# df07/mcp-raytracer

Hardware: AMD Instinct MI355X
Metric: Msamples/sec (w×h×spp/s) Cornell 800×800 spp=256 @1/2/4/8 GPU (higher is better)
Workload: dtype f64

## Files before the change

mcp-raytracer_amd/csrc/pt_kernel.hpp:

```cpp
#pragma once

#include <hip/hip_runtime.h>

#include <cstdint>
#include <type_traits>

#include "rt_math.hpp"
#include "scene.hpp"

namespace rt {

struct DevScene {
    const RtTNode* __restrict__ tnodes;
    const RtPrim* __restrict__ prims;
    const RtPrim* __restrict__ gprims;
    const RtPre* __restrict__ gpre;
    int32_t n_pre;
    const RtExact* __restrict__ xrec;
    int32_t off_xrec;
    const int32_t* __restrict__ tprims;
    const float4* __restrict__ tsph;
    const RtMat* __restrict__ mats;
    const RtLight* __restrict__ lights;
    const RtLight* __restrict__ glights;
// ... 2036 lines not shown
}
__device__ __forceinline__ void item_pixel(const RtRegion& reg, int tiles_x, double rtx, int mt, int l, int& i,
                                           int& j) {
    const int gt = reg.tile_group + mt * reg.tile_groups;
    const int ty = udiv(gt, tiles_x, rtx);
    i = reg.x + (gt - ty * tiles_x) * kTile + (l & (kTile - 1));
    j = reg.y + ty * kTile + (l / kTile);
}
template <class SB>
__device__ __forceinline__ bool slot_pixel(const SB& sb, const RtRegion& reg, int tiles_x, double rtx, int endX,
                                           int endY, int a, int& i, int& j) {
    int ls = a;
    if (sb.act) {
        if (a >= sb.slots) return false;
        ls = sb.act[a];
        __builtin_amdgcn_s_waitcnt(0x0F70);
    }
    item_pixel(reg, tiles_x, rtx, sb.tile0 + (ls >> 6), ls & 63, i, j);
    return i < endX && j < endY;
}

struct PhaseRow {
    int32_t s0, chunk, nch, base;
    double rnch;
    int32_t pad[2];
};
__device__ __forceinline__ void phase_table_init(const SampleBuf& sb, PhaseRow* tab) {
    const int t = threadIdx.x;
    if (t < kMaxPhases) {
        PhaseRow r;
        r.s0 = sb.s0[t];
        r.chunk = sb.chunk[t];
        r.nch = sb.nch[t];
        r.base = t < sb.n_phases ? sb.item_base[t] : 0x7fffffff;
        r.rnch = sb.rnch[t];
        r.pad[0] = r.pad[1] = 0;
        tab[t] = r;
    }
    __syncthreads();
}
__device__ __forceinline__ void item_decode(const SampleBuf& sb, const PhaseRow* tab, int u, int& tl, int& l, int& s,
                                            int& s_end) {
    int ph = 0;
    for (int q = 1; q < sb.n_phases; ++q) ph += u >= tab[q].base ? 1 : 0;
    const PhaseRow r = tab[ph];
    const int v = u - r.base;
    const int q = v >> 6;
    l = v & 63;
    tl = udiv(q, r.nch, r.rnch);
    const int ch = q - tl * r.nch;
    s = r.s0 + ch * r.chunk;
    s_end = s + r.chunk;
}

__device__ __forceinline__ void first_pool(const SampleBuf& sb, int& pool_next, int& pool_end, bool& exhausted) {
    const int gw = (int)(blockIdx.x * (blockDim.x / kWave) + threadIdx.x / kWave);
    pool_next = gw * sb.pool;
    pool_end = min(pool_next + sb.pool, sb.n_items);
    exhausted = pool_next >= sb.n_items;
}
__device__ __forceinline__ void take_pool(const RenderOut& out, const SampleBuf& sb, int lane, int& pool_next,
                                          int& pool_end, bool& exhausted) {
    int base = 0;
    if (lane == 0) base = (int)atomicAdd(out.tile_counter, (unsigned)sb.pool);
    base = __builtin_amdgcn_readfirstlane(__shfl(base, 0, 64)) + (int)(gridDim.x * (blockDim.x / kWave)) * sb.pool;
    if (base >= sb.n_items) {
        exhausted = true;
        return;
    }
    pool_next = base;
    pool_end = min(base + sb.pool, sb.n_items);
}

struct KernArgs {
    DevScene S0;
    RtRegion reg;
    RenderOut out;
    int tiles_x;
    SampleBuf sb;
};
__device__ __forceinline__ const KernArgs& kern_args() {
    KArgPtr p = (KArgPtr)__builtin_amdgcn_kernarg_segment_ptr();
    asm volatile("" : "+s"(p));
    return *(const KernArgs*)p;
}

template <class Real, bool EMIT, int INSTR, int TRAV, int LDSS>
__global__ __launch_bounds__(kBlockChunk) void pt_chunk_kernel(DevScene S0, RtRegion reg, RenderOut out,
                                                                        int tiles_x, SampleBuf sb) {
    constexpr bool COUNT = INSTR == 1;
    constexpr bool PROF = INSTR == 2;
    extern __shared__ int lds_stack[];
    const RtCamera& C0 = S0.cam;
    __shared__ PhaseRow ptab[kMaxPhases];
    phase_table_init(sb, ptab);
    const DevScene S = scene_prologue<LDSS>(S0, lds_stack);
    const int lane = threadIdx.x & (kWave - 1);
    StackT<LDSS>* stk = reinterpret_cast<StackT<LDSS>*>(lds_stack) + threadIdx.x;
    const int endX = min(reg.x + reg.width, C0.width);
    const int endY = min(reg.y + reg.height, C0.height);
    const int n_items = sb.n_items;

    uint32_t cnt[CT_WORDS];
    if (COUNT) {
#pragma unroll
        for (int k = 0; k < CT_WORDS; ++k) cnt[k] = 0;
    }
    unsigned long long st_err = 0;
    __shared__ unsigned long long prof_lds[PROF ? kProfWaves * kProfSlot : 1];
    Prof pf;
    prof_init<PROF>(pf, prof_lds, lane);

    int pool_next, pool_end;
    bool exhausted;
    first_pool(sb, pool_next, pool_end, exhausted);
    int slot = -1;
    int s = 0, s_end = 0, i = 0, j = 0;
    uint32_t pix = 0;
    V3 pc = v3(0, 0, 0);
    bool new_path = false;
    Path<EMIT> P;
    const double rtx = 1.0 / (double)tiles_x;
    constexpr bool RS = trav_fast(TRAV) && INSTR != 1;
    FastWalk<Real> W;
    bool walking = false;
    LaneBounces lb;

#define PK_SB (kern_args().sb)
#define PK_REG (kern_args().reg)
#define PK_OUT (kern_args().out)
#define PK_S (scene_view<LDSS>(kern_args().S0, lds_stack))
    while (true) {
        const unsigned long long need = __ballot(slot < 0);
        const int n_need = __popcll(need);
        if (n_need != 0 && !exhausted && (n_need >= PK_SB.refill_min || __ballot(slot >= 0) == 0ull)) {
            if (pool_next >= pool_end) take_pool(PK_OUT, PK_SB, lane, pool_next, pool_end, exhausted);
            if (!exhausted) {
                const int take = min(n_need, pool_end - pool_next);
                const int rank = __builtin_amdgcn_mbcnt_hi((uint32_t)(need >> 32),
                                                           __builtin_amdgcn_mbcnt_lo((uint32_t)need, 0u));
                if (slot < 0 && rank < take) {
                    int tl, l, s1, e1;
                    item_decode(PK_SB, ptab, pool_next + rank, tl, l, s1, e1);
                    if (slot_pixel(PK_SB, PK_REG, tiles_x, rtx, endX, endY, tl * 64 + l, i, j)) {
                        slot = tl * 64 + l;
                        s = s1;
                        s_end = e1;
                        pix = (uint32_t)j * (uint32_t)C0.width + (uint32_t)i;
                        pc = pixel_center<Real>(cam_opaque(), i, j);
                        new_path = true;
                    }
                }
                pool_next += take;
            }
        }
        psec<PROF>(pf, PR_TILE);
        if (__ballot(slot >= 0) == 0ull) {
            if (exhausted) break;
            continue;
        }
        if constexpr (RS) {
            auto finish_sample = [&](V3 c) {
                rec_put<false>(PK_SB, (size_t)s * PK_SB.stride_s + (size_t)slot * PK_SB.stride_slot, c,
                               P.bounces | rec_err_bits(PK_SB.err_in_rec, st_err), lb, PK_OUT.stats);
                ++s;
                if (s < s_end) new_path = true;
                else slot = -1;
            };
            const RtCamera& C = cam_opaque();
            prof_trip<PROF>(pf);
            if (slot >= 0 && !walking) {
                if (new_path) {
                    path_begin<Real, EMIT>(C, P, pc, pix, (uint32_t)(PK_SB.s_base + s));
                    new_path = false;
                    psec<PROF>(pf, PR_NEWPATH);
                }
                V3 c;
                if (path_pre<Real, EMIT, PROF>(C, P, pf, c)) {
                    finish_sample(c);
                } else {
                    fast_walk_begin<Real, COUNT>(PK_S, P.o, P.d, W, cnt);
                    walking = true;
                }
            }
            psec<PROF>(pf, PR_RR);
            const bool was_walking = walking;
            fast_walk_rounds<Real, COUNT, TRAV == TRAV_FAST_DEFER, PROF, kStackStride, LDSS == 0>(
                PK_S, P.o, P.d, W, walking, stk, PK_SB.min_ready, exhausted, cnt, &pf);
            psec<PROF>(pf, PR_HIT);
            if (was_walking && !walking) {
                fast_walk_resolve<Real, COUNT>(PK_S, P.o, P.d, W, cnt);
                V3 c;
                if (path_post<Real, EMIT, COUNT, PROF>(PK_S, C, P, W.best, W.best_t, cnt, st_err, pf, c))
                    finish_sample(c);
            }
            psec<PROF>(pf, PR_ACC);
        } else if (slot >= 0) {
            const RtCamera& C = cam_opaque();
            prof_trip<PROF>(pf);
            if (new_path) {
                path_begin<Real, EMIT>(C, P, pc, pix, (uint32_t)(PK_SB.s_base + s));
                new_path = false;
                psec<PROF>(pf, PR_NEWPATH);
            }
            V3 c;
            if (path_trip<Real, EMIT, COUNT, PROF, TRAV>(PK_S, C, P, stk, cnt, st_err, pf, c)) {
                rec_put<false>(PK_SB, (size_t)s * PK_SB.stride_s + (size_t)slot * PK_SB.stride_slot, c,
                               P.bounces | rec_err_bits(PK_SB.err_in_rec, st_err), lb, PK_OUT.stats);
                if (COUNT) {
                    cnt[CT_SAMPLES]++;
                    cnt[CT_BOUNCES] += (uint32_t)P.bounces;
                }
                ++s;
                if (s < s_end) new_path = true;
                else slot = -1;
                psec<PROF>(pf, PR_ACC);
            }
        }
    }
    PixStats st;
    lb.to(st);
    publish_stats(out, st, st_err, lane);
    publish_counters<COUNT, PROF>(out, cnt, pf, lane);
#undef PK_SB
#undef PK_REG
#undef PK_OUT
#undef PK_S
}

#ifndef RT_POOL_K
#define RT_POOL_K 152
#endif
#ifndef RT_POOL_PROF
#define RT_POOL_PROF 0
#endif
constexpr int kPoolK = RT_POOL_K;
constexpr int kBlockPool = 1024;
constexpr int kPoolGroups = 3;
static_assert(kPoolK >= kWave && kPoolK <= 256, "pool slots: one full wave, u8 queue entries");
constexpr size_t kPoolWaveBytes = ((size_t)kPoolK * (kPoolGroups * 16 + 8) + 2 * kPoolK + 15) / 16 * 16;
constexpr int kPoolClog2Bits = 3;
constexpr int kPoolMaxChunk = 1 << ((1 << kPoolClog2Bits) - 1);
__device__ __forceinline__ float pool_meta(int phase, int clog2, int mat) {
    return __uint_as_float((uint32_t)((phase + 2) & 0xff) | ((uint32_t)clog2 << 8) | ((uint32_t)mat << 11));
}
__device__ __forceinline__ int meta_phase(float m) { return (int)(__float_as_uint(m) & 0xffu) - 2; }
__device__ __forceinline__ int meta_clog2(float m) { return (int)((__float_as_uint(m) >> 8) & 7u); }
__device__ __forceinline__ int meta_mat(float m) { return (int)(__float_as_uint(m) >> 11); }
__device__ __forceinline__ float pool_hs(int hf16, int s) { return __uint_as_float(((uint32_t)hf16 & 0xffffu) | ((uint32_t)s << 16)); }
__device__ __forceinline__ int hs_s(float v) { return (int)(__float_as_uint(v) >> 16); }
__device__ __forceinline__ int hs_hf(float v) { return (int)(__float_as_uint(v) & 0xffffu); }
__device__ __forceinline__ int item_end(int s, int clog2) { return ((s >> clog2) + 1) << clog2; }
constexpr size_t pool_lds_bytes() { return (size_t)(kBlockPool / kWave) * kPoolWaveBytes; }
enum : int { PH_NEW = -1, PH_ITEM = -2 };

__device__ __forceinline__ void stack_push(uint8_t* q, bool top, int& cnt, bool want, int k) {
    const unsigned long long m = __ballot(want);
    if (want) {
        const int r = __builtin_amdgcn_mbcnt_hi((uint32_t)(m >> 32), __builtin_amdgcn_mbcnt_lo((uint32_t)m, 0u));
        q[top ? kPoolK - 1 - (cnt + r) : cnt + r] = (uint8_t)k;
    }
    cnt += __popcll(m);
}

struct KernArgsPrimary {
    KernArgs args;
    const uint2* ptab;
};
__device__ __forceinline__ const uint2* primary_table_opaque() {
    KArgPtr p = (KArgPtr)__builtin_amdgcn_kernarg_segment_ptr();
    asm volatile("" : "+s"(p));
    return *(const uint2* const*)(p + offsetof(KernArgsPrimary, ptab));
}

template <class Real, int TRAV, int LDSS, bool PRIM>
__device__ __forceinline__ void pool_trips(DevScene S0, RtRegion reg, RenderOut out, int tiles_x, SampleBuf sb) {
    extern __shared__ int lds_stack[];
    const RtCamera& C0 = S0.cam;
    __shared__ PhaseRow ptab[kMaxPhases];
    phase_table_init(sb, ptab);
    const DevScene S = scene_prologue<LDSS>(S0, lds_stack);
    const int lane = threadIdx.x & (kWave - 1);
    StackT<LDSS>* stk = reinterpret_cast<StackT<LDSS>*>(lds_stack) + threadIdx.x;
    char* wpool = reinterpret_cast<char*>(lds_stack) + S0.lds_pool_off + (size_t)(threadIdx.x / kWave) * kPoolWaveBytes;
    float4* G = reinterpret_cast<float4*>(wpool);
    float2* G3 = reinterpret_cast<float2*>(wpool + (size_t)kPoolK * kPoolGroups * 16);
    uint8_t* qa = reinterpret_cast<uint8_t*>(wpool + (size_t)kPoolK * (kPoolGroups * 16 + 8));
    uint8_t* qd = qa + kPoolK;
    const int endX = min(reg.x + reg.width, C0.width);
    const int endY = min(reg.y + reg.height, C0.height);
    const int n_items = sb.n_items;
    const double rtx = 1.0 / (double)tiles_x;
    uint32_t* cnt = nullptr;
    unsigned long long st_err = 0;
    constexpr bool PP = RT_POOL_PROF;
    __shared__ unsigned long long prof_lds[PP ? kProfWaves * kProfSlot : 1];
    Prof pf;
    prof_init<PP>(pf, prof_lds, lane);

    for (int k = lane; k < kPoolK; k += kWave) {
        qa[k] = (uint8_t)k;
        G[k] = make_float4(0.f, 0.f, pool_meta(PH_ITEM, 0, 0), 0.f);
    }
    int a_cnt = kPoolK, d_cnt = 0;
    int dl_cnt = 0;
    int an_cnt = kPoolK, ac_cnt = 0;
    int pool_next, pool_end;
    bool exhausted;
    first_pool(sb, pool_next, pool_end, exhausted);

    LaneBounces lb;
    auto record = [&](V3 c, int bounces, int slot, int& s, int s_end, unsigned long long err = 0ull) -> int {
        if (!sb.err_in_rec) st_err |= err;
        rec_put<true>(sb, (size_t)s * sb.stride_s + (size_t)slot * sb.stride_slot, c,
                           bounces | (sb.err_in_rec ? (int)((uint32_t)err << kRecErrShift) : 0), lb, out.stats);
        ++s;
        return s < s_end ? PH_NEW : PH_ITEM;
    };

    while (a_cnt + d_cnt + dl_cnt > 0) {
        __asm__ volatile("" ::: "memory");
        prof_trip<PP>(pf);
        psec<PP>(pf, PR_ACC);
        const bool dtop = dl_cnt > d_cnt;
        const int dn = dtop ? dl_cnt : d_cnt;
        const bool atop = ac_cnt > an_cnt;
        const int an = atop ? ac_cnt : an_cnt;
        if (dn >= kWave || dn > an) {
            const int n = min(kWave, dn);
            int k = -1, phase = 0;
            if (lane < n) k = (int)qd[dtop ? kPoolK - dl_cnt + lane : d_cnt - n + lane];
            if (dtop) dl_cnt -= n;
            else d_cnt -= n;
            if (k >= 0) {
                const float4 g0 = G[k], g1 = G[kPoolK + k], g2 = G[2 * kPoolK + k];
                const float2 g3 = G3[k];
                Path<false> P;
                P.rng = (uint64_t)__float_as_uint(g0.x) | ((uint64_t)__float_as_uint(g0.y) << 32);
                P.bounces = meta_phase(g0.z);
                P.em_n = 0;
                P.o = V3{g1.x, g1.y, g1.z};
                P.d = V3{g2.x, g2.y, g2.z};
                P.T = V3{g2.w, g3.x, g3.y};
                const int hf = hs_hf(g0.w);
                const int h = hf & 0x3fff;
                const bool planar = (hf >> 14) & 1, front = (hf >> 15) & 1;
                const V3 att = ld3(S.mats[meta_mat(g0.z)].color);
                const int clog2 = meta_clog2(g0.z), slot = __float_as_int(g1.w);
                int s = hs_s(g0.w);
                const int s_end = item_end(s, clog2);
                phase = P.bounces;
                const RtCamera& C = cam_opaque();
                const bool dterm =
                    dtop ? shade_diffuse<Real, false, false, PP, 2>(S, C, P, h, planar, front, P.o, P.d, att, cnt, pf)
                         : shade_diffuse<Real, false, false, PP, 1>(S, C, P, h, planar, front, P.o, P.d, att, cnt, pf);
                if (dterm) {
                    const V3 c = mulv(ld3(S.mats[S.prims[h].mat].emitted), P.T);
                    phase = record(c, P.bounces, slot, s, s_end);
                }
                G[k] = make_float4(__uint_as_float((uint32_t)P.rng), __uint_as_float((uint32_t)(P.rng >> 32)),
                                   pool_meta(phase, clog2, 0), pool_hs(0, s));
                G[2 * kPoolK + k] = make_float4(P.d.x, P.d.y, P.d.z, P.T.x);
                G3[k] = make_float2(P.T.y, P.T.z);
            }
            stack_push(qa, false, an_cnt, k >= 0 && phase < 0, k);
            stack_push(qa, true, ac_cnt, k >= 0 && phase >= 0, k);
            a_cnt = an_cnt + ac_cnt;
        } else {
            const int n = min(kWave, an);
            int k = -1;
            if (lane < n) k = (int)qa[atop ? kPoolK - ac_cnt + lane : an_cnt - n + lane];
            if (atop) ac_cnt -= n;
            else an_cnt -= n;
            a_cnt -= n;
            float4 g0 = make_float4(0.f, 0.f, pool_meta(PH_ITEM, 0, 0), 0.f), g1 = g0, g2 = g0;
            float2 g3 = make_float2(0.f, 0.f);
            if (k >= 0) {
                g0 = G[k];
                g1 = G[kPoolK + k];
                g2 = G[2 * kPoolK + k];
                g3 = G3[k];
            }
            int phase = meta_phase(g0.z), clog2 = meta_clog2(g0.z), slot = __float_as_int(g1.w);
            int s = hs_s(g0.w);
            const unsigned long long need = __ballot(k >= 0 && phase == PH_ITEM);
            if (need != 0ull && !exhausted) {
                if (pool_next >= pool_end) take_pool(out, sb, lane, pool_next, pool_end, exhausted);
                if (!exhausted) {
                    const int take = min(__popcll(need), pool_end - pool_next);
                    const int rank = __builtin_amdgcn_mbcnt_hi((uint32_t)(need >> 32),
                                                               __builtin_amdgcn_mbcnt_lo((uint32_t)need, 0u));
                    if (k >= 0 && phase == PH_ITEM && rank < take) {
                        int tl, l, s1, e1, i, j;
                        item_decode(sb, ptab, pool_next + rank, tl, l, s1, e1);
                        if (slot_pixel(sb, reg, tiles_x, rtx, endX, endY, tl * 64 + l, i, j)) {
                            slot = tl * 64 + l;
                            s = s1;
                            clog2 = __builtin_ctz((uint32_t)(e1 - s1));
                            phase = PH_NEW;
                        }
                    }
                    pool_next += take;
                }
            }
            const bool keep = k >= 0 && (phase != PH_ITEM || !exhausted);
            bool to_d = false, d_light = false;
            if (k >= 0 && phase != PH_ITEM) {
                const RtCamera& C = cam_opaque();
                Path<false> P;
                uint2 prec = make_uint2(0u, 0u);
                if (phase == PH_NEW) {
                    int i, j;
                    slot_pixel(sb, reg, tiles_x, rtx, endX, endY, slot, i, j);
                    const uint32_t pix = (uint32_t)j * (uint32_t)C.width + (uint32_t)i;
                    if (PRIM) prec = primary_table_opaque()[pix];
                    path_begin<Real, false>(C, P, pixel_center<Real>(C, i, j), pix, (uint32_t)(sb.s_base + s));
                    if (PRIM) __builtin_amdgcn_s_waitcnt(0x0F70);
                } else {
                    P.rng = (uint64_t)__float_as_uint(g0.x) | ((uint64_t)__float_as_uint(g0.y) << 32);
                    P.o = V3{g1.x, g1.y, g1.z};
                    P.d = V3{g2.x, g2.y, g2.z};
                    P.T = V3{g2.w, g3.x, g3.y};
                    P.bounces = phase;
                    P.em_n = 0;
                }
                V3 c;
                psec<PP>(pf, PR_NEWPATH);
                bool term = path_pre<Real, false, PP>(C, P, pf, c);
                V3 att;
                int hf = 0, dmat = 0;
                unsigned long long err = 0ull;
                if (!term) {
                    const RayK<Real> ray = make_ray<Real>(P.o, P.d);
                    Real t;
                    int h;
                    if (PRIM && !atop) {
                        psec<PP>(pf, PR_TILE);
                        h = closest_hit_primary<Real, false>(S, ray, t, prec, cnt);
                    } else if (PP && TRAV == TRAV_BRUTE && C.n_prims <= kBruteMaxPrims)
                        h = closest_hit_brute_nf<Real, false>(S, C.n_prims, ray, t, lot_column(stk), cnt,
                                                              [&]() { psec<PP>(pf, PR_TILE); });
                    else
                        h = closest_hit_any<Real, false, TRAV>(S, C.n_prims, ray, t, stk, cnt);
                    psec<PP>(pf, PR_HIT);
                    if (h < 0) {
                        term = true;
                        c = miss_color<Real, false, PP>(C, P, err, pf);
                    } else {
                        V3 p, nrm, emitted, sdir;
                        bool front, planar;
                        const int kind = shade_hit<Real, false, false, PP>(S, P, h, t, cnt, pf, p, nrm, front,
                                                                              planar, emitted, att, sdir, &dmat);
                        if (kind == SC_NONE) {
                            term = true;
                            c = emitted;
                        } else {
                            ++P.bounces;
                            P.o = p;
                            if (kind == SC_SPEC) {
                                P.T = mulv(P.T, att);
                                P.d = sdir;
                            } else {
                                to_d = true;
                                P.d = nrm;
                                hf = h | (planar ? (1 << 14) : 0) | (front ? (1 << 15) : 0);
                                {
                                    uint64_t r = P.rng;
                                    const Real u0 = uniform<Real>(r);
                                    const Real rnd = S.mix_total == 1.0 ? u0 : u0 * (Real)S.mix_total;
                                    d_light = !(rnd < (Real)0.5 || C.n_lights == 0);
                                }
                            }
                        }
                    }
                }
                phase = term ? record(c, P.bounces, slot, s, item_end(s, clog2), err) : P.bounces;
                g0 = make_float4(__uint_as_float((uint32_t)P.rng), __uint_as_float((uint32_t)(P.rng >> 32)),
                                 pool_meta(phase, clog2, to_d ? dmat : 0), pool_hs(to_d ? hf : 0, s));
                g1 = make_float4(P.o.x, P.o.y, P.o.z, __int_as_float(slot));
                g2 = make_float4(P.d.x, P.d.y, P.d.z, P.T.x);
                g3 = make_float2(P.T.y, P.T.z);
            } else if (keep) {
                g0 = make_float4(0.f, 0.f, pool_meta(PH_ITEM, 0, 0), 0.f);
            }
            if (keep) {
                G[k] = g0;
                G[kPoolK + k] = g1;
                G[2 * kPoolK + k] = g2;
                G3[k] = g3;
            }
            stack_push(qa, false, an_cnt, keep && !to_d && phase < 0, k);
            stack_push(qa, true, ac_cnt, keep && !to_d && phase >= 0, k);
            a_cnt = an_cnt + ac_cnt;
            stack_push(qd, false, d_cnt, to_d && !d_light, k);
            stack_push(qd, true, dl_cnt, to_d && d_light, k);
        }
    }
    PixStats st;
    lb.to(st);
    publish_stats(out, st, st_err, lane);
    publish_counters<false, PP>(out, cnt, pf, lane);
}

template <class Real, int TRAV, int LDSS>
__global__ __launch_bounds__(kBlockPool) void pt_pool_kernel(DevScene S0, RtRegion reg, RenderOut out, int tiles_x,
                                                               SampleBuf sb) {
    pool_trips<Real, TRAV, LDSS, false>(S0, reg, out, tiles_x, sb);
}
template <class Real, int TRAV, int LDSS>
__global__ __launch_bounds__(kBlockPool) void pt_pool_primary_kernel(DevScene S0, RtRegion reg, RenderOut out,
                                                                       int tiles_x, SampleBuf sb, const uint2* ptab) {
    (void)ptab;
    pool_trips<Real, TRAV, LDSS, true>(S0, reg, out, tiles_x, sb);
}

}
```

Measured before the change: 13410.

## Merge diffuse and continuation path queues into one per-trip wave schedule

The wavefront pool loop used to run either a diffuse-shading batch or an active-path batch on each trip. Now a diffuse batch is topped up with continuing active paths so all lanes stay busy, and after diffuse shading those lanes go straight on to trace their next ray in the same trip. New-path fetching keeps its own batch type. The aim is fewer idle lanes and fewer loop trips, at the cost of more divergence within a wave and higher register pressure from the unified body.

Measured after the change: 13770 (median of 6 runs). 1.03x the previous value.

```diff
diff --git a/mcp-raytracer_amd/csrc/pt_kernel.hpp b/mcp-raytracer_amd/csrc/pt_kernel.hpp
--- a/mcp-raytracer_amd/csrc/pt_kernel.hpp
+++ b/mcp-raytracer_amd/csrc/pt_kernel.hpp
@@ -2362,8 +2362,7 @@
         qa[k] = (uint8_t)k;
         G[k] = make_float4(0.f, 0.f, pool_meta(PH_ITEM, 0, 0), 0.f);
     }
-    int a_cnt = kPoolK, d_cnt = 0;
-    int dl_cnt = 0;
+    int d_cnt = 0, dl_cnt = 0;
     int an_cnt = kPoolK, ac_cnt = 0;
     int pool_next, pool_end;
     bool exhausted;
@@ -2378,71 +2377,56 @@
         return s < s_end ? PH_NEW : PH_ITEM;
     };
 
-    while (a_cnt + d_cnt + dl_cnt > 0) {
+    enum : int { FR_N, FR_D, FR_NONE };
+    while (an_cnt + ac_cnt + d_cnt + dl_cnt > 0) {
         __asm__ volatile("" ::: "memory");
         prof_trip<PP>(pf);
         psec<PP>(pf, PR_ACC);
         const bool dtop = dl_cnt > d_cnt;
         const int dn = dtop ? dl_cnt : d_cnt;
-        const bool atop = ac_cnt > an_cnt;
-        const int an = atop ? ac_cnt : an_cnt;
-        if (dn >= kWave || dn > an) {
-            const int n = min(kWave, dn);
-            int k = -1, phase = 0;
-            if (lane < n) k = (int)qd[dtop ? kPoolK - dl_cnt + lane : d_cnt - n + lane];
-            if (dtop) dl_cnt -= n;
-            else d_cnt -= n;
-            if (k >= 0) {
-                const float4 g0 = G[k], g1 = G[kPoolK + k], g2 = G[2 * kPoolK + k];
-                const float2 g3 = G3[k];
-                Path<false> P;
-                P.rng = (uint64_t)__float_as_uint(g0.x) | ((uint64_t)__float_as_uint(g0.y) << 32);
-                P.bounces = meta_phase(g0.z);
-                P.em_n = 0;
-                P.o = V3{g1.x, g1.y, g1.z};
-                P.d = V3{g2.x, g2.y, g2.z};
-                P.T = V3{g2.w, g3.x, g3.y};
-                const int hf = hs_hf(g0.w);
-                const int h = hf & 0x3fff;
-                const bool planar = (hf >> 14) & 1, front = (hf >> 15) & 1;
-                const V3 att = ld3(S.mats[meta_mat(g0.z)].color);
-                const int clog2 = meta_clog2(g0.z), slot = __float_as_int(g1.w);
-                int s = hs_s(g0.w);
-                const int s_end = item_end(s, clog2);
-                phase = P.bounces;
-                const RtCamera& C = cam_opaque();
-                const bool dterm =
-                    dtop ? shade_diffuse<Real, false, false, PP, 2>(S, C, P, h, planar, front, P.o, P.d, att, cnt, pf)
-                         : shade_diffuse<Real, false, false, PP, 1>(S, C, P, h, planar, front, P.o, P.d, att, cnt, pf);
-                if (dterm) {
-                    const V3 c = mulv(ld3(S.mats[S.prims[h].mat].emitted), P.T);
-                    phase = record(c, P.bounces, slot, s, s_end);
-                }
-                G[k] = make_float4(__uint_as_float((uint32_t)P.rng), __uint_as_float((uint32_t)(P.rng >> 32)),
-                                   pool_meta(phase, clog2, 0), pool_hs(0, s));
-                G[2 * kPoolK + k] = make_float4(P.d.x, P.d.y, P.d.z, P.T.x);
-                G3[k] = make_float2(P.T.y, P.T.z);
-            }
-            stack_push(qa, false, an_cnt, k >= 0 && phase < 0, k);
-            stack_push(qa, true, ac_cnt, k >= 0 && phase >= 0, k);
-            a_cnt = an_cnt + ac_cnt;
+        const int fr = dn >= kWave       ? FR_D
+                       : ac_cnt >= kWave ? FR_NONE
+                       : an_cnt >= kWave ? FR_N
+                       : dn > 0          ? FR_D
+                       : an_cnt > 0      ? FR_N
+                                         : FR_NONE;
+        int k = -1;
+        int nd = 0;
+        if (fr == FR_D) {
+            nd = min(kWave, dn);
+            const int na = min(kWave - nd, ac_cnt);
+            if (lane < nd) k = (int)qd[dtop ? kPoolK - dl_cnt + lane : d_cnt - nd + lane];
+            else if (lane < nd + na) k = (int)qa[kPoolK - ac_cnt + lane - nd];
+            if (dtop) dl_cnt -= nd;
+            else d_cnt -= nd;
+            ac_cnt -= na;
+        } else if (fr == FR_N) {
+            const int n = min(kWave, an_cnt);
+            if (lane < n) k = (int)qa[an_cnt - n + lane];
+            an_cnt -= n;
         } else {
-            const int n = min(kWave, an);
-            int k = -1;
-            if (lane < n) k = (int)qa[atop ? kPoolK - ac_cnt + lane : an_cnt - n + lane];
-            if (atop) ac_cnt -= n;
-            else an_cnt -= n;
-            a_cnt -= n;
-            float4 g0 = make_float4(0.f, 0.f, pool_meta(PH_ITEM, 0, 0), 0.f), g1 = g0, g2 = g0;
-            float2 g3 = make_float2(0.f, 0.f);
-            if (k >= 0) {
-                g0 = G[k];
-                g1 = G[kPoolK + k];
-                g2 = G[2 * kPoolK + k];
-                g3 = G3[k];
-            }
-            int phase = meta_phase(g0.z), clog2 = meta_clog2(g0.z), slot = __float_as_int(g1.w);
-            int s = hs_s(g0.w);
+            const int n = min(kWave, ac_cnt);
+            if (lane < n) k = (int)qa[kPoolK - ac_cnt + lane];
+            ac_cnt -= n;
+        }
+        float4 g0 = make_float4(0.f, 0.f, pool_meta(PH_ITEM, 0, 0), 0.f), g1 = g0, g2 = g0;
+        float2 g3 = make_float2(0.f, 0.f);
+        if (k >= 0) {
+            g0 = G[k];
+            g1 = G[kPoolK + k];
+            g2 = G[2 * kPoolK + k];
+            g3 = G3[k];
+        }
+        int phase = meta_phase(g0.z), clog2 = meta_clog2(g0.z), slot = __float_as_int(g1.w);
+        int s = hs_s(g0.w);
+        const RtCamera& C = cam_opaque();
+        Path<false> P;
+        bool keep = k >= 0;
+        bool path = false;
+        bool term = false;
+        V3 c = v3(0, 0, 0);
+        uint2 prec = make_uint2(0u, 0u);
+        if (fr == FR_N) {
             const unsigned long long need = __ballot(k >= 0 && phase == PH_ITEM);
             if (need != 0ull && !exhausted) {
                 if (pool_next >= pool_end) take_pool(out, sb, lane, pool_next, pool_end, exhausted);
@@ -2463,98 +2447,116 @@
                     pool_next += take;
                 }
             }
-            const bool keep = k >= 0 && (phase != PH_ITEM || !exhausted);
-            bool to_d = false, d_light = false;
-            if (k >= 0 && phase != PH_ITEM) {
-                const RtCamera& C = cam_opaque();
-                Path<false> P;
-                uint2 prec = make_uint2(0u, 0u);
-                if (phase == PH_NEW) {
-                    int i, j;
-                    slot_pixel(sb, reg, tiles_x, rtx, endX, endY, slot, i, j);
-                    const uint32_t pix = (uint32_t)j * (uint32_t)C.width + (uint32_t)i;
-                    if (PRIM) prec = primary_table_opaque()[pix];
-                    path_begin<Real, false>(C, P, pixel_center<Real>(C, i, j), pix, (uint32_t)(sb.s_base + s));
-                    if (PRIM) __builtin_amdgcn_s_waitcnt(0x0F70);
+            keep = k >= 0 && (phase != PH_ITEM || !exhausted);
+            if (k >= 0 && phase == PH_NEW) {
+                path = true;
+                int i, j;
+                slot_pixel(sb, reg, tiles_x, rtx, endX, endY, slot, i, j);
+                const uint32_t pix = (uint32_t)j * (uint32_t)C.width + (uint32_t)i;
+                if (PRIM) prec = primary_table_opaque()[pix];
+                path_begin<Real, false>(C, P, pixel_center<Real>(C, i, j), pix, (uint32_t)(sb.s_base + s));
+                if (PRIM) __builtin_amdgcn_s_waitcnt(0x0F70);
+            }
+            psec<PP>(pf, PR_NEWPATH);
+        } else {
+            if (k >= 0) {
+                path = true;
+                P.rng = (uint64_t)__float_as_uint(g0.x) | ((uint64_t)__float_as_uint(g0.y) << 32);
+                P.o = V3{g1.x, g1.y, g1.z};
+                P.d = V3{g2.x, g2.y, g2.z};
+                P.T = V3{g2.w, g3.x, g3.y};
+                P.bounces = phase;
+                P.em_n = 0;
+            }
+            if (fr == FR_D) {
+                if (lane < nd) {
+                    const int hf = hs_hf(g0.w);
+                    const int h = hf & 0x3fff;
+                    const bool planar = (hf >> 14) & 1, front = (hf >> 15) & 1;
+                    const V3 att = ld3(S.mats[meta_mat(g0.z)].color);
+                    const bool dterm =
+                        dtop ? shade_diffuse<Real, false, false, PP, 2>(S, C, P, h, planar, front, P.o, P.d, att, cnt, pf)
+                             : shade_diffuse<Real, false, false, PP, 1>(S, C, P, h, planar, front, P.o, P.d, att, cnt, pf);
+                    if (dterm) {
+                        term = true;
+                        c = mulv(ld3(S.mats[S.prims[h].mat].emitted), P.T);
+                    }
+                }
+            } else {
+                psec<PP>(pf, PR_NEWPATH);
+            }
+        }
+        bool to_d = false, d_light = false;
+        int hf = 0, dmat = 0;
+        unsigned long long err = 0ull;
+        if (path && !term) {
+            term = path_pre<Real, false, PP>(C, P, pf, c);
+            if (!term) {
+                const RayK<Real> ray = make_ray<Real>(P.o, P.d);
+                Real t;
+                int h;
+                V3 att;
+                if (PRIM && fr == FR_N) {
+                    psec<PP>(pf, PR_TILE);
+                    h = closest_hit_primary<Real, false>(S, ray, t, prec, cnt);
+                } else if (PP && TRAV == TRAV_BRUTE && C.n_prims <= kBruteMaxPrims)
+                    h = closest_hit_brute_nf<Real, false>(S, C.n_prims, ray, t, lot_column(stk), cnt,
+                                                          [&]() { psec<PP>(pf, PR_TILE); });
+                else
+                    h = closest_hit_any<Real, false, TRAV>(S, C.n_prims, ray, t, stk, cnt);
+                psec<PP>(pf, PR_HIT);
+                if (h < 0) {
+                    term = true;
+                    c = miss_color<Real, false, PP>(C, P, err, pf);
                 } else {
-                    P.rng = (uint64_t)__float_as_uint(g0.x) | ((uint64_t)__float_as_uint(g0.y) << 32);
-                    P.o = V3{g1.x, g1.y, g1.z};
-                    P.d = V3{g2.x, g2.y, g2.z};
-                    P.T = V3{g2.w, g3.x, g3.y};
-                    P.bounces = phase;
-                    P.em_n = 0;
-                }
-                V3 c;
-                psec<PP>(pf, PR_NEWPATH);
-                bool term = path_pre<Real, false, PP>(C, P, pf, c);
-                V3 att;
-                int hf = 0, dmat = 0;
-                unsigned long long err = 0ull;
-                if (!term) {
-                    const RayK<Real> ray = make_ray<Real>(P.o, P.d);
-                    Real t;
-                    int h;
-                    if (PRIM && !atop) {
-                        psec<PP>(pf, PR_TILE);
-                        h = closest_hit_primary<Real, false>(S, ray, t, prec, cnt);
-                    } else if (PP && TRAV == TRAV_BRUTE && C.n_prims <= kBruteMaxPrims)
-                        h = closest_hit_brute_nf<Real, false>(S, C.n_prims, ray, t, lot_column(stk), cnt,
-                                                              [&]() { psec<PP>(pf, PR_TILE); });
-                    else
-                        h = closest_hit_any<Real, false, TRAV>(S, C.n_prims, ray, t, stk, cnt);
-                    psec<PP>(pf, PR_HIT);
-                    if (h < 0) {
+                    V3 p, nrm, emitted, sdir;
+                    bool front, planar;
+                    const int kind = shade_hit<Real, false, false, PP>(S, P, h, t, cnt, pf, p, nrm, front, planar,
+                                                                          emitted, att, sdir, &dmat);
+                    if (kind == SC_NONE) {
                         term = true;
-                        c = miss_color<Real, false, PP>(C, P, err, pf);
+                        c = emitted;
                     } else {
-                        V3 p, nrm, emitted, sdir;
-                        bool front, planar;
-                        const int kind = shade_hit<Real, false, false, PP>(S, P, h, t, cnt, pf, p, nrm, front,
-                                                                              planar, emitted, att, sdir, &dmat);
-                        if (kind == SC_NONE) {
-                            term = true;
-                            c = emitted;
+                        ++P.bounces;
+                        P.o = p;
+                        if (kind == SC_SPEC) {
+                            P.T = mulv(P.T, att);
+                            P.d = sdir;
                         } else {
-                            ++P.bounces;
-                            P.o = p;
-                            if (kind == SC_SPEC) {
-                                P.T = mulv(P.T, att);
-                                P.d = sdir;
-                            } else {
-                                to_d = true;
-                                P.d = nrm;
-                                hf = h | (planar ? (1 << 14) : 0) | (front ? (1 << 15) : 0);
-                                {
-                                    uint64_t r = P.rng;
-                                    const Real u0 = uniform<Real>(r);
-                                    const Real rnd = S.mix_total == 1.0 ? u0 : u0 * (Real)S.mix_total;
-                                    d_light = !(rnd < (Real)0.5 || C.n_lights == 0);
-                                }
+                            to_d = true;
+                            P.d = nrm;
+                            hf = h | (planar ? (1 << 14) : 0) | (front ? (1 << 15) : 0);
+                            {
+                                uint64_t r = P.rng;
+                                const Real u0 = uniform<Real>(r);
+                                const Real rnd = S.mix_total == 1.0 ? u0 : u0 * (Real)S.mix_total;
+                                d_light = !(rnd < (Real)0.5 || C.n_lights == 0);
                             }
                         }
                     }
                 }
-                phase = term ? record(c, P.bounces, slot, s, item_end(s, clog2), err) : P.bounces;
-                g0 = make_float4(__uint_as_float((uint32_t)P.rng), __uint_as_float((uint32_t)(P.rng >> 32)),
-                                 pool_meta(phase, clog2, to_d ? dmat : 0), pool_hs(to_d ? hf : 0, s));
-                g1 = make_float4(P.o.x, P.o.y, P.o.z, __int_as_float(slot));
-                g2 = make_float4(P.d.x, P.d.y, P.d.z, P.T.x);
-                g3 = make_float2(P.T.y, P.T.z);
-            } else if (keep) {
-                g0 = make_float4(0.f, 0.f, pool_meta(PH_ITEM, 0, 0), 0.f);
-            }
-            if (keep) {
-                G[k] = g0;
-                G[kPoolK + k] = g1;
-                G[2 * kPoolK + k] = g2;
-                G3[k] = g3;
-            }
-            stack_push(qa, false, an_cnt, keep && !to_d && phase < 0, k);
-            stack_push(qa, true, ac_cnt, keep && !to_d && phase >= 0, k);
-            a_cnt = an_cnt + ac_cnt;
-            stack_push(qd, false, d_cnt, to_d && !d_light, k);
-            stack_push(qd, true, dl_cnt, to_d && d_light, k);
-        }
+            }
+        }
+        if (path) {
+            phase = term ? record(c, P.bounces, slot, s, item_end(s, clog2), err) : P.bounces;
+            g0 = make_float4(__uint_as_float((uint32_t)P.rng), __uint_as_float((uint32_t)(P.rng >> 32)),
+                             pool_meta(phase, clog2, to_d ? dmat : 0), pool_hs(to_d ? hf : 0, s));
+            g1 = make_float4(P.o.x, P.o.y, P.o.z, __int_as_float(slot));
+            g2 = make_float4(P.d.x, P.d.y, P.d.z, P.T.x);
+            g3 = make_float2(P.T.y, P.T.z);
+        } else if (keep) {
+            g0 = make_float4(0.f, 0.f, pool_meta(PH_ITEM, 0, 0), 0.f);
+        }
+        if (keep) {
+            G[k] = g0;
+            G[kPoolK + k] = g1;
+            G[2 * kPoolK + k] = g2;
+            G3[k] = g3;
+        }
+        stack_push(qa, false, an_cnt, keep && !to_d && phase < 0, k);
+        stack_push(qa, true, ac_cnt, keep && !to_d && phase >= 0, k);
+        stack_push(qd, false, d_cnt, to_d && !d_light, k);
+        stack_push(qd, true, dl_cnt, to_d && d_light, k);
     }
     PixStats st;
     lb.to(st);
```
